# theouterlimitz/Audio-Mastering-Engine

Hardware: NVIDIA B200
Metric: audio-sec mastered/sec (x realtime) (higher is better)
Workload: dtype f64

## Files before the change

### audio_mastering_engine_b200/csrc/ame.cu

```cuda
#include <algorithm>
#include <cmath>
#include <cstdarg>
#include <cstdio>
#include <cstring>
#include <dlfcn.h>
#include <mutex>
#include <string>
#include <vector>

#include "ame_kernels.cuh"

using namespace ame;

namespace {

thread_local std::string g_err;

int fail(int code, const char *fmt, ...) {
    char buf[512];
    va_list ap;
    va_start(ap, fmt);
    vsnprintf(buf, sizeof buf, fmt, ap);
    va_end(ap);
    g_err = buf;
// ... 114 lines not shown
    std::vector<Slot> slots;
    double *d_energy = nullptr;
    int *d_chain_stats = nullptr;
    long long *d_hist = nullptr;
    int *d_hist_st = nullptr;
    int *d_peak = nullptr;
    unsigned *d_tp = nullptr;
    int *d_lim_stats = nullptr;
    int lim_guess = -1;
    ame_track_result *d_results = nullptr;
    KwJob *d_meter_kw = nullptr;
    GainJob *d_meter_peak = nullptr;
    int32_t *d_meter_tracks = nullptr;
    TrackDev *d_meter_tdev = nullptr;
    double *d_meter_energy = nullptr;
    int *d_meter_sp = nullptr;
    unsigned *d_meter_tp = nullptr;
    ame_loudness *d_loud_out = nullptr;
    ame_loudness *d_loud_any = nullptr;
    cudaStream_t s_in = nullptr, s_out = nullptr;
    std::vector<cudaEvent_t> ev_in, ev_run;
    std::vector<cudaEvent_t> ev_meter;
    bool timing = false;
    int t_step = -1, t_wave = 0;
    std::vector<cudaEvent_t> t_ev;
    std::vector<char> t_used;
    std::vector<cudaEvent_t> tl_ev;
    int tl_waves = 0;
};

namespace {

inline bool t_on(const ame_plan *p) {
    return p->timing && p->t_step >= 0 && p->t_step < kMaxTimedSteps && p->t_wave < kMaxTimedWaves;
}
inline size_t t_slot(const ame_plan *p, int kernel) {
    return ((size_t)p->t_step * kMaxTimedWaves + p->t_wave) * AME_N_KERNELS + kernel;
}
inline void t_begin(ame_plan *p, int kernel, cudaStream_t s) {
    if (t_on(p)) cudaEventRecord(p->t_ev[t_slot(p, kernel) * 2], s);
}
inline void t_end(ame_plan *p, int kernel, cudaStream_t s) {
    if (t_on(p)) {
        cudaEventRecord(p->t_ev[t_slot(p, kernel) * 2 + 1], s);
        p->t_used[t_slot(p, kernel)] = 1;
    }
}

int plan_alloc(ame_plan *p, void **ptr, size_t bytes) {
    *ptr = nullptr;
    if (bytes == 0) return AME_OK;
    cudaError_t e = dev_alloc(ptr, bytes);
    if (e != cudaSuccess) {
        *ptr = nullptr;
        return fail(AME_E_NOMEM, "device allocation of %zu bytes failed: %s", bytes, cudaGetErrorString(e));
    }
    p->allocs.push_back(*ptr);
    return AME_OK;
}

int dmalloc(ame_plan *p, void **ptr, size_t bytes) {
    const int rc = plan_alloc(p, ptr, bytes);
    if (rc == AME_OK) p->ws_bytes += bytes;
    return rc;
}

template <class T>
int upload(ame_plan *p, T **dptr, const std::vector<T> &v) {
    if (int rc = plan_alloc(p, (void **)dptr, v.size() * sizeof(T))) return rc;
    if (!v.empty()) CU(cudaMemcpy(*dptr, v.data(), v.size() * sizeof(T), cudaMemcpyHostToDevice));
    return AME_OK;
}

#define LAUNCH_CHECK(p)                                                                            \
    do {                                                                                           \
        cudaError_t e_ = cudaGetLastError();                                                       \
        if (e_ != cudaSuccess) return fail(AME_E_CUDA, "kernel launch failed: %s (%s:%d)", cudaGetErrorString(e_), __FILE__, __LINE__); \
        ++(p)->launches;                                                                           \
    } while (0)

int check_warmth(const ame_plan *p) {
    for (int t = 0; t < p->n_tracks; ++t)
        if (p->tracks[t].flags & AME_F_WARMTH) {
            const int l = p->tracks[t].warm_lut;
            if (l < 0 || l >= p->n_luts) return fail(AME_E_INVALID, "track %d needs warmth table %d but %d are set", t, l, p->n_luts);
        }
    return AME_OK;
}

struct Bufs {
    const int16_t *in = nullptr;
    int16_t *pre = nullptr, *bands = nullptr, *out = nullptr;
    uint16_t *rms = nullptr, *list = nullptr;
    int *tile_cnt = nullptr, *n_flagged = nullptr;
    GrpRec *grp = nullptr;
    double *att = nullptr;
    int64_t *hist = nullptr;
    int16_t *norm = nullptr;
    long long *lim_last = nullptr;
    LimStore lim_in{}, lim_out{};
    int *lim_need = nullptr;
};

Bufs slot_bufs(ame_plan *p, const Wave &w, const int16_t *d_in, int16_t *d_out) {
    const Slot &sl = p->slots[w.slot];
    Bufs b;
    b.in = d_in; b.out = d_out;
    b.pre = sl.pre - 2 * w.frame_lo;
    b.bands = sl.bands; b.rms = sl.rms; b.list = sl.list; b.tile_cnt = sl.tile_cnt; b.n_flagged = sl.n_flagged;
    b.grp = sl.grp; b.att = sl.att;
    b.norm = sl.norm ? sl.norm - 2 * w.frame_lo : nullptr;
    b.lim_last = sl.lim_last; b.lim_in = sl.lim_in; b.lim_out = sl.lim_out; b.lim_need = sl.lim_need;
    b.hist = (int64_t *)p->d_hist;
    return b;
}

int run_eq(ame_plan *p, const Wave &w, const int16_t *d_in, int16_t *d_pre, cudaStream_t s) {
    if (!w.eq.n) return AME_OK;
    t_begin(p, S_EQ, s);
    if (p->precision == 1)
        k_eq_f32<<<(w.eq.n + 127) / 128, 128, 0, s>>>(p->d_eq_jobs + w.eq.lo, w.eq.n, p->d_tracks, p->d_luts, d_in, d_pre);
    else
        k_eq<<<(w.eq.n + kEqBlock - 1) / kEqBlock, kEqBlock, 0, s>>>(p->d_eq_jobs + w.eq.lo, w.eq.n, p->d_tracks, p->d_luts, d_in, d_pre);
    LAUNCH_CHECK(p);
    t_end(p, S_EQ, s);
    return AME_OK;
}

int run_split(ame_plan *p, const Wave &w, const int16_t *d_pre, int16_t *d_bands, cudaStream_t s) {
    if (!w.split.n) return AME_OK;
    t_begin(p, S_SPLIT, s);
    if (w.xover_uni)
        k_band_split<true><<<(w.split.n + 127) / 128, 128, 0, s>>>(w.xover, p->d_split_jobs + w.split.lo, w.split.n, p->d_tracks, p->d_mb_delta,
                                                                   d_pre, d_bands, p->mb_frames);
    else
        k_band_split<false><<<(w.split.n + 127) / 128, 128, 0, s>>>(w.xover, p->d_split_jobs + w.split.lo, w.split.n, p->d_tracks, p->d_mb_delta,
                                                                    d_pre, d_bands, p->mb_frames);
    LAUNCH_CHECK(p);
    t_end(p, S_SPLIT, s);
    return AME_OK;
}

int chain_lanes(const ame_plan *p, int n_chains) {
    if (p->chain_warps < 0) return 1;
    if (p->chain_warps > 0) return 32 * p->chain_warps;
    if (n_chains * 2 <= p->n_sm) return 256;
    return (n_chains >= p->n_sm && p->slots.size() > 1) ? 64 : 128;
}

int run_compress(ame_plan *p, const Wave &w, const Bufs &b, cudaStream_t s) {
    if (!w.chain.n) return AME_OK;
    t_begin(p, S_FLAG, s);
    int *tile_base = b.tile_cnt + std::max(p->slot_tiles, 1);
    k_window_flag<<<w.wf.n, kWfThreads, 0, s>>>(p->d_wf_jobs + w.wf.lo, b.bands, b.rms, b.tile_cnt, b.grp);
    LAUNCH_CHECK(p);
    k_tile_prefix<<<w.chain.n, kWfThreads, 0, s>>>(p->d_chain_jobs + w.chain.lo, b.tile_cnt, tile_base, b.n_flagged);
    LAUNCH_CHECK(p);
    k_compact<<<(w.wf.n + kWfThreads / 32 - 1) / (kWfThreads / 32), kWfThreads, 0, s>>>(p->d_wf_jobs + w.wf.lo, w.wf.n, b.rms, b.tile_cnt,
                                                                                          tile_base, b.list, b.grp);
    LAUNCH_CHECK(p);
    t_end(p, S_FLAG, s);
    t_begin(p, S_CHAIN, s);
    const int lanes = chain_lanes(p, w.chain.n);
    k_att_chain<<<w.chain.n, std::max(lanes, 32), 0, s>>>(p->d_chain_jobs + w.chain.lo, b.list, b.n_flagged, p->d_tables, b.att, p->mb_frames,
                                            lanes, p->d_chain_stats + 2 * (size_t)w.chain.lo);
    LAUNCH_CHECK(p);
    t_end(p, S_CHAIN, s);
    t_begin(p, S_APPLY, s);
    k_compress_apply<<<(unsigned)((w.seg_hi - w.seg_lo + 3) / 4), 128, 0, s>>>(p->d_mb_chunks + w.mb_chunks.lo, w.mb_chunks.n, w.seg_lo, w.seg_hi,
                                                                                b.bands, b.grp, b.att, b.pre, p->mb_frames);
    LAUNCH_CHECK(p);
    t_end(p, S_APPLY, s);
    return AME_OK;
}

int run_hist(ame_plan *p, const Wave &w, const int16_t *d_pre, int64_t *d_hist, cudaStream_t s) {
    const int nt = w.track_hi - w.track_lo;
    if (nt <= 0) return AME_OK;
    CU(cudaMemsetAsync(p->d_peak + w.track_lo, 0, (size_t)nt * 4, s));
    if (w.kw.n) {
        t_begin(p, S_KW, s);
        if (w.kw_uni)
            k_kweight_energy<true><<<(w.kw.n + 127) / 128, 128, 0, s>>>(w.kw_cfg, p->d_kw_jobs + w.kw.lo, w.kw.n, p->d_tracks, p->d_tdev, d_pre,
                                                                        p->d_energy, p->d_peak);
        else
            k_kweight_energy<false><<<(w.kw.n + 127) / 128, 128, 0, s>>>(w.kw_cfg, p->d_kw_jobs + w.kw.lo, w.kw.n, p->d_tracks, p->d_tdev, d_pre,
                                                                         p->d_energy, p->d_peak);
        LAUNCH_CHECK(p);
        t_end(p, S_KW, s);
    }
    t_begin(p, S_TAIL, s);
    k_tail_peak<<<nt, 128, 0, s>>>(p->d_tracks, p->d_tdev, w.track_lo, w.track_hi, d_pre, p->d_peak);
    LAUNCH_CHECK(p);
    t_end(p, S_TAIL, s);
    CU(cudaMemsetAsync(p->d_tp + w.track_lo, 0, (size_t)nt * 4, s));
    if (w.true_peak && w.gain.n) {
        t_begin(p, S_TP, s);
        k_true_peak<<<w.gain.n, 256, 0, s>>>(p->d_gain_jobs + w.gain.lo, p->d_tracks, d_pre, p->d_tp);
        LAUNCH_CHECK(p);
        t_end(p, S_TP, s);
    }
    t_begin(p, S_HIST, s);
    k_block_hist<<<nt, 256, 0, s>>>(p->d_tdev, w.track_lo, p->d_energy, (long long *)d_hist, p->d_hist_st);
    LAUNCH_CHECK(p);
    t_end(p, S_HIST, s);
    return AME_OK;
}

int run_apply(ame_plan *p, const Wave &w, const int16_t *d_pre, int16_t *d_out, const Bufs &b, cudaStream_t s) {
    int16_t *d_norm = b.norm;
    long long *lim_last = b.lim_last;
    if (!w.gain.n) return AME_OK;
    t_begin(p, S_GAIN, s);
    if (w.limiter) CU(cudaMemsetAsync(lim_last, 0xff, (size_t)w.lim.n * sizeof(long long), s));
    k_apply_gain<<<w.gain.n, 256, 0, s>>>(p->d_gain_jobs + w.gain.lo, p->d_results, p->d_tracks, p->d_tdev, d_pre, d_out, d_norm, lim_last);
    LAUNCH_CHECK(p);
    t_end(p, S_GAIN, s);
    if (w.limiter) {
        t_begin(p, S_LIM, s);
        const GainJob *gj = p->d_lim_jobs + w.lim.lo;
        constexpr int kLimRounds = 2;
        int cap = 64;
        while (cap < p->lim_keep + 2) cap *= 2;
        const size_t smem = lim_smem_bytes(cap);
        for (int round = 0; round <= kLimRounds; ++round) {
            if (round == 0) {
                k_limiter<<<w.lim.n, 256, smem, s>>>(gj, w.lim.n, lim_last, p->d_tracks, d_norm, d_out, b.lim_in, b.lim_out, b.lim_need, 0, cap, p->lim_guess);
                LAUNCH_CHECK(p);
            }
            k_limiter<<<w.lim.n, 32, smem, s>>>(gj, w.lim.n, lim_last, p->d_tracks, d_norm, d_out, b.lim_in, b.lim_out, b.lim_need, round, cap, p->lim_guess);
            LAUNCH_CHECK(p);
            k_lim_verify<<<(w.lim.n + 3) / 4, 128, 0, s>>>(gj, w.lim.n, p->d_tracks, b.lim_in, b.lim_out, b.lim_need,
                                                             p->d_lim_stats + round);
            LAUNCH_CHECK(p);
        }
        k_lim_fallback<<<w.lim.n, 32, smem, s>>>(gj, w.lim.n, p->d_tracks, d_norm, d_out, b.lim_in, b.lim_out, b.lim_need, cap);
        LAUNCH_CHECK(p);
        t_end(p, S_LIM, s);
    }
    return AME_OK;
}

int run_gain(ame_plan *p, const Wave &w, const int16_t *d_pre, const int64_t *d_hist, int16_t *d_out, const Bufs &b, cudaStream_t s) {
    const int nt = w.track_hi - w.track_lo;
    if (nt <= 0) return AME_OK;
    t_begin(p, S_FIN, s);
    k_finalize<<<nt, 128, 0, s>>>(p->d_tracks, w.track_lo, w.track_hi, (const long long *)d_hist, p->d_hist_st, p->d_peak,
                                             p->d_tp, p->d_results);
    LAUNCH_CHECK(p);
    t_end(p, S_FIN, s);
    return run_apply(p, w, d_pre, d_out, b, s);
}

int run_meter(ame_plan *p, const Wave &w, const int16_t *buf, ame_loudness *res, cudaStream_t s) {
    if (!w.meter_tracks.n) return AME_OK;
    const int nt = w.track_hi - w.track_lo;
    CU(cudaMemsetAsync(p->d_meter_sp + w.track_lo, 0, (size_t)nt * 4, s));
    CU(cudaMemsetAsync(p->d_meter_tp + w.track_lo, 0, (size_t)nt * 4, s));
    if (w.meter_kw.n) {
        if (w.kw_uni)
            k_kweight_energy<true><<<(w.meter_kw.n + 127) / 128, 128, 0, s>>>(w.kw_cfg, p->d_meter_kw + w.meter_kw.lo, w.meter_kw.n, p->d_tracks,
                                                                              p->d_meter_tdev, buf, p->d_meter_energy, p->d_meter_sp);
        else
            k_kweight_energy<false><<<(w.meter_kw.n + 127) / 128, 128, 0, s>>>(w.kw_cfg, p->d_meter_kw + w.meter_kw.lo, w.meter_kw.n, p->d_tracks,
                                                                               p->d_meter_tdev, buf, p->d_meter_energy, p->d_meter_sp);
        LAUNCH_CHECK(p);
    }
    if (w.meter_peak.n) {
        k_meter_peak<<<w.meter_peak.n, 256, 0, s>>>(p->d_meter_peak + w.meter_peak.lo, p->d_tracks, buf, p->d_meter_tp, p->d_meter_sp);
        LAUNCH_CHECK(p);
    }
    k_meter_finalize<<<w.meter_tracks.n, 256, 0, s>>>(p->d_meter_tracks + w.meter_tracks.lo, p->d_tracks, p->d_meter_tdev, p->d_meter_energy,
                                                      p->d_meter_sp, p->d_meter_tp, res);
    LAUNCH_CHECK(p);
    return AME_OK;
}

int run_measure(ame_plan *p, const Wave &w, const Bufs &b, cudaStream_t s) {
    int rc;
    if ((rc = run_eq(p, w, b.in, b.pre, s))) return rc;
    if ((rc = run_split(p, w, b.pre, b.bands, s))) return rc;
    if ((rc = run_compress(p, w, b, s))) return rc;
    return run_hist(p, w, b.pre, b.hist, s);
}

int run_chain_of_stages(ame_plan *p, const Wave &w, const Bufs &b, cudaStream_t s) {
    int rc = run_measure(p, w, b, s);
    if (rc) return rc;
    return run_gain(p, w, b.pre, b.hist, b.out, b, s);
}

int drain(ame_plan *p, int rc) {
    (void)p;
    if (rc != AME_OK) cudaDeviceSynchronize();
    return rc;
}

}

extern "C" {

int ame_abi_version(void) { return AME_ABI_VERSION; }
size_t ame_sizeof_track_params(void) { return sizeof(ame_track_params); }
size_t ame_sizeof_track_result(void) { return sizeof(ame_track_result); }
size_t ame_sizeof_plan_options(void) { return sizeof(ame_plan_options); }
size_t ame_sizeof_loudness(void) { return sizeof(ame_loudness); }
const char *ame_last_error(void) { return g_err.c_str(); }
// ... 615 lines not shown
```

### audio_mastering_engine_b200/csrc/ame_kernels.cuh

```cuda
#pragma once
#include <cuda_runtime.h>
#include <stdint.h>
#include "ame_layout.h"

namespace ame {

constexpr unsigned kFull = 0xffffffffu;

__constant__ double c_hist_bounds[1001];
__constant__ double c_hist_energy[1000];

__device__ __forceinline__ uint4 ldg16(const uint4 *p) { return __ldg(p); }

__device__ __forceinline__ double bq_step(const ame_biquad &c, double &z0, double &z1, double x) {
    double y = fma(c.b0, x, z0);
    z0 = fma(-c.a1, y, fma(c.b1, x, z1));
    z1 = fma(-c.a2, y, c.b2 * x);
    return y;
}

__device__ __forceinline__ double i16_to_f64(int x) {
    return __hiloint2double(0x43300000, (int)(0x80000000u ^ (unsigned)x)) - 4503601774854144.0;
}

// ... 162 lines not shown
    auto fetch_lut = [&](const uint4 &q, double *l, double *r) {
        const uint32_t w[4] = {q.x, q.y, q.z, q.w};
#pragma unroll
        for (int k = 0; k < 4; ++k) {
            l[k] = __ldg(lut + (int)(int16_t)(w[k] & 0xffffu));
            r[k] = __ldg(lut + (int)(int16_t)(w[k] >> 16));
        }
    };
    if (WARM) fetch_lut(cur, lutL, lutR);
    constexpr int LAG = (SKEW && MASK != 0) ? 1 : 0;
    for (int it = 0; it < n_it + LAG; ++it) {
        uint4 nn = nxt;
        if (it + 2 < n_it) nn = ldg16(src + it + 2);
        double nL[4] = {0, 0, 0, 0}, nR[4] = {0, 0, 0, 0};
        if (WARM) fetch_lut(nxt, nL, nR);
        const int64_t g = g0f + 4 * (int64_t)(it - LAG);
        const uint32_t w[4] = {cur.x, cur.y, cur.z, cur.w};
        uint32_t o[4];
#pragma unroll
        for (int k = 0; k < 4; ++k) o[k] = frame(w[k], lutL[k], lutR[k]);
        if (it < LAG) {
        } else if (g >= job.tile_begin && g + 4 <= f_hi) {
            dst[it - LAG] = make_uint4(o[0], o[1], o[2], o[3]);
        } else {
#pragma unroll
            for (int k = 0; k < 4; ++k)
                if (g + k >= job.tile_begin && g + k < f_hi) reinterpret_cast<uint32_t *>(dst + it - LAG)[k] = o[k];
        }
        cur = nxt; nxt = nn;
#pragma unroll
        for (int k = 0; k < 4; ++k) { lutL[k] = nL[k]; lutR[k] = nR[k]; }
    }
}

#define AME_EQ_KERNEL(NAME, F, SK)                                                                                  \
__global__ void __launch_bounds__(256, 1)                                                                          \
NAME(const TileJob *__restrict__ jobs, int n_jobs, const ame_track_params *__restrict__ tracks,                    \
     const double *__restrict__ luts, const int16_t *__restrict__ in, int16_t *__restrict__ pre) {                 \
    const int j = blockIdx.x * blockDim.x + threadIdx.x;                                                           \
    if (j >= n_jobs) return;                                                                                       \
    const TileJob job = jobs[j];                                                                                   \
    if (job.tile_end <= job.tile_begin) return;                          \
    const ame_track_params *tp = tracks + job.track;                                                               \
    switch (job.variant) {                                                 \
        AME_EQ_CASE(0, F, SK) AME_EQ_CASE(1, F, SK) AME_EQ_CASE(2, F, SK) AME_EQ_CASE(3, F, SK) AME_EQ_CASE(4, F, SK)    \
        AME_EQ_CASE(5, F, SK) AME_EQ_CASE(6, F, SK) AME_EQ_CASE(7, F, SK) AME_EQ_CASE(8, F, SK) AME_EQ_CASE(9, F, SK)    \
        AME_EQ_CASE(10, F, SK) AME_EQ_CASE(11, F, SK) AME_EQ_CASE(12, F, SK) AME_EQ_CASE(13, F, SK) AME_EQ_CASE(14, F, SK) \
        AME_EQ_CASE(15, F, SK)                                                                                     \
    }                                                                                                              \
}
#define AME_EQ_CASE(M, F, SK) case M: eq_tile<M, false, F, SK>(job, tp, luts, in, pre); break; \
                              case M + 16: eq_tile<M, true, F, SK>(job, tp, luts, in, pre); break;
AME_EQ_KERNEL(k_eq, double, false)
AME_EQ_KERNEL(k_eq_f32, float, false)
#undef AME_EQ_CASE
#undef AME_EQ_KERNEL

template <bool UNI>
__global__ void __launch_bounds__(128, 3)
k_band_split(const __grid_constant__ XoverCfg xc, const TileJob *__restrict__ jobs, int n_jobs, const ame_track_params *__restrict__ tracks,
             const int64_t *__restrict__ mb_delta,
             const int16_t *__restrict__ pre, int16_t *__restrict__ bands, int64_t mb_frames) {
    const int j = blockIdx.x * blockDim.x + threadIdx.x;
    if (j >= n_jobs) return;
    const TileJob job = jobs[j];
    const ame_track_params *tp = tracks + job.track;
    const double lb0 = UNI ? xc.lb0 : tp->xlp[0].b0, la10 = UNI ? xc.la10 : tp->xlp[0].a1, la20 = UNI ? xc.la20 : tp->xlp[0].a2,
                 la11 = UNI ? xc.la11 : tp->xlp[1].a1, la21 = UNI ? xc.la21 : tp->xlp[1].a2;
    const double hb0 = UNI ? xc.hb0 : tp->xhp[0].b0, ha10 = UNI ? xc.ha10 : tp->xhp[0].a1, ha20 = UNI ? xc.ha20 : tp->xhp[0].a2,
                 ha11 = UNI ? xc.ha11 : tp->xhp[1].a1, ha21 = UNI ? xc.ha21 : tp->xhp[1].a2;
    const int64_t delta = mb_delta[job.track];
    double zl[8], zr[8];
#pragma unroll
    for (int i = 0; i < 8; ++i) { zl[i] = 0.0; zr[i] = 0.0; }
    int64_t f_lo = job.tile_begin - (int64_t)tp->warm_xover;
    if (f_lo < job.chunk_begin) f_lo = job.chunk_begin;
    const int64_t f_hi = job.tile_end;
    if (f_hi <= f_lo) return;
    const int64_t g0f = f_lo & ~(int64_t)7;
    const int n_it = (int)((f_hi - g0f + 7) >> 3);
    uint32_t *b0 = reinterpret_cast<uint32_t *>(bands) + delta;
    uint32_t *b1 = b0 + mb_frames;
    uint32_t *b2 = b1 + mb_frames;

    auto split = [&](int xm, double *z, int &p0, int &p1, int &p2) {
        const double x = i16_to_unit(xm);
        const double lo = bw_step1<1, double>(la11, la21, z[2], z[3], bw_step<1, double>(lb0, la10, la20, z[0], z[1], x));
        const double hi = bw_step1<-1, double>(ha11, ha21, z[6], z[7], bw_step<-1, double>(hb0, ha10, ha20, z[4], z[5], x));
        const double mid = __dsub_rn(__dsub_rn(x, lo), hi);
        p0 = to_pcm_f64(lo); p1 = to_pcm_f64(mid); p2 = to_pcm_f64(hi);
    };

    const uint4 *src = reinterpret_cast<const uint4 *>(pre) + (g0f >> 2);
    uint4 c0 = ldg16(src), c1 = ldg16(src + 1), n0 = make_uint4(0, 0, 0, 0), n1 = n0;
    {
        uint32_t *cw0 = reinterpret_cast<uint32_t *>(&c0), *cw1 = reinterpret_cast<uint32_t *>(&c1);
#pragma unroll
        for (int k = 0; k < 4; ++k) {
            if (g0f + k < job.chunk_begin) cw0[k] = 0;
            if (g0f + 4 + k < job.chunk_begin) cw1[k] = 0;
        }
    }
    if (n_it > 1) { n0 = ldg16(src + 2); n1 = ldg16(src + 3); }
    for (int it = 0; it < n_it; ++it) {
        uint4 m0 = n0, m1 = n1;
        if (it + 2 < n_it) { m0 = ldg16(src + 2 * it + 4); m1 = ldg16(src + 2 * it + 5); }
        const int64_t g = g0f + 8 * (int64_t)it;
        const uint32_t w[8] = {c0.x, c0.y, c0.z, c0.w, c1.x, c1.y, c1.z, c1.w};
        uint32_t o0[8], o1[8], o2[8];
#pragma unroll
        for (int k = 0; k < 8; ++k) {
            int l0, l1, l2, r0, r1, r2;
            split((int)(int16_t)(w[k] & 0xffffu), zl, l0, l1, l2);
            split((int)(int16_t)(w[k] >> 16), zr, r0, r1, r2);
            o0[k] = pack16(l0, r0); o1[k] = pack16(l1, r1); o2[k] = pack16(l2, r2);
        }
        if (g >= job.tile_begin && g + 8 <= f_hi) {
            uint4 *q0 = reinterpret_cast<uint4 *>(b0 + g), *q1 = reinterpret_cast<uint4 *>(b1 + g), *q2 = reinterpret_cast<uint4 *>(b2 + g);
            q0[0] = make_uint4(o0[0], o0[1], o0[2], o0[3]); q0[1] = make_uint4(o0[4], o0[5], o0[6], o0[7]);
            q1[0] = make_uint4(o1[0], o1[1], o1[2], o1[3]); q1[1] = make_uint4(o1[4], o1[5], o1[6], o1[7]);
            q2[0] = make_uint4(o2[0], o2[1], o2[2], o2[3]); q2[1] = make_uint4(o2[4], o2[5], o2[6], o2[7]);
        } else {
#pragma unroll
            for (int k = 0; k < 8; ++k)
                if (g + k >= job.tile_begin && g + k < f_hi) { b0[g + k] = o0[k]; b1[g + k] = o1[k]; b2[g + k] = o2[k]; }
        }
        c0 = n0; c1 = n1; n0 = m0; n1 = m1;
    }
}

__device__ __forceinline__ unsigned energy_of(uint32_t w) {
    const int l = (int16_t)(w & 0xffffu), r = (int16_t)(w >> 16);
    return (unsigned)(l * l) + (unsigned)(r * r);
}

__device__ __forceinline__ void load8(const uint32_t *__restrict__ p, int64_t idx, int64_t lo, int64_t hi, uint32_t *w) {
    if (idx >= lo && idx + 8 <= hi && ((reinterpret_cast<uintptr_t>(p + idx) & 15) == 0)) {
        const uint4 a = __ldg(reinterpret_cast<const uint4 *>(p + idx));
        const uint4 b = __ldg(reinterpret_cast<const uint4 *>(p + idx) + 1);
        w[0] = a.x; w[1] = a.y; w[2] = a.z; w[3] = a.w; w[4] = b.x; w[5] = b.y; w[6] = b.z; w[7] = b.w;
    } else {
#pragma unroll
        for (int k = 0; k < 8; ++k) w[k] = (idx + k >= lo && idx + k < hi) ? __ldg(p + idx + k) : 0u;
    }
}

__device__ __forceinline__ unsigned isqrt_ratio(unsigned long long s, unsigned n) {
    unsigned r = (unsigned)__fsqrt_rn(__fdividef((float)s, (float)n));
    if ((unsigned long long)r * r * n > s) --r;
    else if ((unsigned long long)(r + 1) * (r + 1) * n <= s) ++r;
    return r;
}

__global__ void __launch_bounds__(kWfThreads)
k_window_flag(const WfJob *__restrict__ jobs, const int16_t *__restrict__ bands, uint16_t *__restrict__ rms,
              int *__restrict__ tile_cnt, GrpRec *__restrict__ grp) {
    __shared__ long long s_scan[kWfThreads / 32];
    __shared__ unsigned long long s_head[kWfThreads / 32];
    __shared__ int s_flag[kWfThreads / 32];
    const WfJob job = jobs[blockIdx.x];
    const uint32_t *bp = reinterpret_cast<const uint32_t *>(bands) + job.plane_off;
    uint16_t *rp = rms + job.plane_off;
    const int64_t n = job.n, t0 = job.tile_begin;
    const int look = job.look;
    const int lane = threadIdx.x & 31, wid = threadIdx.x >> 5;
    const int64_t i0 = t0 + (int64_t)threadIdx.x * 8;
    uint32_t w[8], wo[8];
    load8(bp, i0, 0, n, w);
    load8(bp, i0 - look, 0, n, wo);
    unsigned long long head = 0;
    for (int64_t j = t0 - look + threadIdx.x; j < t0; j += kWfThreads)
        if (j >= 0) head += energy_of(__ldg(bp + j));
#pragma unroll
    for (int d = 16; d > 0; d >>= 1) head += __shfl_xor_sync(kFull, head, d);
    if (lane == 0) s_head[wid] = head;
    long long pre[8];
    long long run = 0;
#pragma unroll
    for (int k = 0; k < 8; ++k) {
        pre[k] = run;
        run += (long long)energy_of(w[k]) - (long long)energy_of(wo[k]);
    }
    long long incl = run;
#pragma unroll
    for (int d = 1; d < 32; d <<= 1) {
        const long long v = __shfl_up_sync(kFull, incl, d);
        if (lane >= d) incl += v;
    }
    if (lane == 31) s_scan[wid] = incl;
    __syncthreads();
    long long base = incl - run;
    unsigned long long h = 0;
#pragma unroll
    for (int q = 0; q < kWfThreads / 32; ++q) {
        if (q < wid) base += s_scan[q];
        h += s_head[q];
    }
    base += (long long)h;
    const unsigned long long thr2 = (unsigned long long)job.thr_i * job.thr_i;
    const bool never = job.thr_i > 32768u;
    uint32_t o[4] = {0, 0, 0, 0};
    unsigned m8 = 0;
    if (t0 >= look && i0 + 8 <= n) {
        const unsigned long long bound = thr2 * (unsigned long long)(2 * look);
#pragma unroll
        for (int k = 0; k < 8; ++k) {
            const unsigned long long s = (unsigned long long)(base + pre[k]);
            unsigned r = 0;
            if (!never && s >= bound) r = isqrt_ratio(s, (unsigned)(2 * look));
            m8 |= (r != 0 ? 1u : 0u) << k;
            o[k >> 1] |= (r & 0xffffu) << ((k & 1) * 16);
        }
    } else {
#pragma unroll
        for (int k = 0; k < 8; ++k) {
            const int64_t i = i0 + k;
            const long long s = base + pre[k];
            const int64_t nfr = i < look ? i : look;
            unsigned r = 0;
            if (!never && i < n && nfr > 0 && (unsigned long long)s >= thr2 * (unsigned long long)(2 * nfr))
                r = isqrt_ratio((unsigned long long)s, (unsigned)(2 * nfr));
            m8 |= (r != 0 ? 1u : 0u) << k;
            o[k >> 1] |= (r & 0xffffu) << ((k & 1) * 16);
        }
    }
    const int cnt = __popc(m8);
    int fincl = cnt;
#pragma unroll
    for (int d = 1; d < 32; d <<= 1) {
        const int v = __shfl_up_sync(kFull, fincl, d);
        if (lane >= d) fincl += v;
    }
    if (lane == 31) s_flag[wid] = fincl;
    const unsigned m1 = __shfl_down_sync(kFull, m8, 1), m2 = __shfl_down_sync(kFull, m8, 2), m3 = __shfl_down_sync(kFull, m8, 3);
    __syncthreads();
    int fbase = 0, total = 0;
#pragma unroll
    for (int q = 0; q < kWfThreads / 32; ++q) {
        if (q < wid) fbase += s_flag[q];
        total += s_flag[q];
    }
    const int rank = fbase + fincl - cnt;
    if ((threadIdx.x & 3) == 0 && i0 < n)
        grp[job.grp_begin + (i0 >> 5)] = GrpRec{m8 | (m1 << 8) | (m2 << 16) | (m3 << 24), (uint32_t)rank};
    if (m8) {
        uint16_t *dp = rp + t0 + rank;
        int slot = 0;
#pragma unroll
        for (int k = 0; k < 8; ++k)
            if (m8 & (1u << k)) dp[slot++] = (uint16_t)((o[k >> 1] >> ((k & 1) * 16)) & 0xffffu);
    }
    if (threadIdx.x == 0) tile_cnt[blockIdx.x] = total;
}

__device__ __forceinline__ double att_update(double att, double m, double inc, double dec, double tau) {
    const long long ia = __double_as_longlong(att);
    const bool above = ia > __double_as_longlong(m);
    const bool rising = ia < __double_as_longlong(tau);
    const double s = att + inc;
    const double d = att - dec;
    const double r = above ? d : m;
    return (rising && !above) ? s : r;
}

struct RmsBlk { uint32_t w[4]; };

__device__ __forceinline__ RmsBlk list_load(const uint16_t *__restrict__ lp, int64_t i, int64_t lim, bool vec) {
    RmsBlk q;
    q.w[0] = q.w[1] = q.w[2] = q.w[3] = 0;
    if (vec && i + 8 <= lim) {
        const uint4 v = __ldg(reinterpret_cast<const uint4 *>(lp + i));
        q.w[0] = v.x; q.w[1] = v.y; q.w[2] = v.z; q.w[3] = v.w;
    } else if (i < lim) {
#pragma unroll
        for (int k = 0; k < 8; ++k)
            if (i + k < lim) q.w[k >> 1] |= (uint32_t)__ldg(lp + i + k) << ((k & 1) * 16);
    }
    return q;
}

__global__ void __launch_bounds__(kWfThreads)
k_tile_prefix(const ChainJob *__restrict__ jobs, const int *__restrict__ tile_cnt, int *__restrict__ tile_base,
              int *__restrict__ n_flagged) {
    __shared__ int s_warp[kWfThreads / 32];
    const ChainJob job = jobs[blockIdx.x];
    const int n_tiles = (int)((job.n + kWfTile - 1) / kWfTile);
    const int t = threadIdx.x, lane = t & 31, wid = t >> 5;
    int carry = 0;
    for (int j0 = 0; j0 < n_tiles; j0 += kWfThreads) {
        const int j = j0 + t;
        const int c = j < n_tiles ? tile_cnt[job.tile0 + j] : 0;
        int incl = c;
#pragma unroll
        for (int d = 1; d < 32; d <<= 1) {
            const int v = __shfl_up_sync(kFull, incl, d);
            if (lane >= d) incl += v;
        }
        if (lane == 31) s_warp[wid] = incl;
        __syncthreads();
        int base = carry, total = 0;
#pragma unroll
        for (int q = 0; q < kWfThreads / 32; ++q) {
            if (q < wid) base += s_warp[q];
            total += s_warp[q];
        }
        if (j < n_tiles) tile_base[job.tile0 + j] = base + incl - c;
        carry += total;
        __syncthreads();
    }
    if (t == 0) n_flagged[blockIdx.x] = carry;
}

__global__ void __launch_bounds__(kWfThreads)
k_compact(const WfJob *__restrict__ jobs, int n_tiles, const uint16_t *__restrict__ rms, const int *__restrict__ tile_cnt,
          const int *__restrict__ tile_base, uint16_t *__restrict__ list, GrpRec *__restrict__ grp) {
    const int lane = threadIdx.x & 31;
    const int tile = blockIdx.x * (kWfThreads / 32) + (threadIdx.x >> 5);
    if (tile >= n_tiles) return;
    const WfJob job = jobs[tile];
    const int cnt = tile_cnt[tile], base = tile_base[tile];
    if (base) {
        const int64_t frames = min((int64_t)kWfTile, job.n - job.tile_begin);
        const int ng = (int)((frames + 31) >> 5);
        GrpRec *gr = grp + job.grp_begin + (job.tile_begin >> 5);
        for (int g = lane; g < ng; g += 32) gr[g].base += (uint32_t)base;
    }
    const uint16_t *rp = rms + job.plane_off + job.tile_begin;
    uint16_t *lp = list + job.plane_off + base;
    for (int j = lane; j < cnt; j += 32) lp[j] = rp[j];
}


__device__ __forceinline__ void list_entries(AttEntry *e, const AttEntry *tbl, const RmsBlk &q) {
#pragma unroll
    for (int k = 0; k < 8; ++k) {
        const unsigned r = (q.w[k >> 1] >> ((k & 1) * 16)) & 0xffffu;
        asm("ld.global.nc.v4.f64 {%0,%1,%2,%3}, [%4];" : "=d"(e[k].m), "=d"(e[k].inc), "=d"(e[k].dec), "=d"(e[k].tau) : "l"(tbl + r));
    }
}

struct SegSum {
    long long margin;
    long long at_p;
    long long lo, hi;
    int64_t p;
    int exp0;
    bool open;
    bool ok;
};

__device__ __forceinline__ void segsum_begin(SegSum &u, double start) {
    u.margin = 0x7fffffffffffffffLL; u.at_p = 0; u.lo = 0; u.hi = -1; u.p = 0;
    u.exp0 = (int)(__double_as_longlong(start) >> 52);
    u.open = true; u.ok = u.exp0 > 0;
}

template <bool DUAL>
__device__ __forceinline__ bool list_step8(const AttEntry *e, double *al, int64_t i, int64_t lim, bool avec, double &a, double &b,
                                           SegSum &u, double &max_m, double &sum_dec) {
    double o[8];
#pragma unroll
    for (int k = 0; k < 8; ++k) {
        if (!DUAL) { max_m = fmax(max_m, e[k].m); sum_dec += e[k].dec; }
        if (DUAL && u.open && i + k < lim) {
            const long long ib = __double_as_longlong(b), im = __double_as_longlong(e[k].m);
            if (ib > im) {
                u.margin = min(u.margin, ib - im);
                const long long id = __double_as_longlong(e[k].dec);
                if (id != 0) {
                    const int ed = (int)(id >> 52);
                    const long long mant = (id & 0xfffffffffffffLL) | (ed ? (1LL << 52) : 0LL);
                    if ((ed ? ed : 1) + (__ffsll(mant) - 1) == u.exp0 - 1) u.ok = false;
                }
                ++u.p;
            } else {
                u.open = false;
                u.at_p = ib; u.lo = __double_as_longlong(e[k].tau); u.hi = im;
                if ((int)(ib >> 52) != u.exp0) u.ok = false;
            }
        }
        b = att_update(b, e[k].m, e[k].inc, e[k].dec, e[k].tau);
        if (DUAL) a = att_update(a, e[k].m, e[k].inc, e[k].dec, e[k].tau);
        o[k] = b;
    }
    if (avec && i + 8 <= lim) {
        double2 *d = reinterpret_cast<double2 *>(al + i);
        d[0] = make_double2(o[0], o[1]); d[1] = make_double2(o[2], o[3]);
        d[2] = make_double2(o[4], o[5]); d[3] = make_double2(o[6], o[7]);
    } else {
#pragma unroll
        for (int k = 0; k < 8; ++k)
            if (i + k < lim) al[i + k] = o[k];
    }
    return DUAL && __double_as_longlong(a) == __double_as_longlong(b);
}

template <bool DUAL>
__device__ __forceinline__ bool list_walk(const uint16_t *lp, const AttEntry *tbl, double *al, int64_t b0, int64_t b1, bool vec,
                                          bool avec, double a, double &b, SegSum &u, double &max_m, double &sum_dec) {
    if (b0 >= b1) return false;
    RmsBlk r0 = list_load(lp, b0, b1, vec), r1 = list_load(lp, b0 + 8, b1, vec);
    AttEntry ea[8], eb[8];
    list_entries(ea, tbl, r0);
    for (int64_t i = b0; i < b1; i += 16) {
        r0 = list_load(lp, i + 16, b1, vec);
// ... 867 lines not shown
```

Before: 932,100.

## Process each window-flag tile with a single warp looping over rows

Rewrites k_window_flag so that one warp handles a whole tile by looping in 256-sample rows. Prefix sums and flag counts carry across rows in registers instead of going through shared memory and __syncthreads. The next row's loads are prefetched while the current row is scanned. A monotone threshold test also skips the isqrt when the running sum is below the bound. The risks are a serial loop per warp, fewer blocks per tile, and a new 'wide' fallback path for the -32768 sample case.

New measurement: 958,800 (median of 6 runs). 2.9% higher.

```diff
diff --git a/audio_mastering_engine_b200/csrc/ame.cu b/audio_mastering_engine_b200/csrc/ame.cu
--- a/audio_mastering_engine_b200/csrc/ame.cu
+++ b/audio_mastering_engine_b200/csrc/ame.cu
@@ -290,7 +290,8 @@
     if (!w.chain.n) return AME_OK;
     t_begin(p, S_FLAG, s);
     int *tile_base = b.tile_cnt + std::max(p->slot_tiles, 1);
-    k_window_flag<<<w.wf.n, kWfThreads, 0, s>>>(p->d_wf_jobs + w.wf.lo, b.bands, b.rms, b.tile_cnt, b.grp);
+    k_window_flag<<<(w.wf.n + kWfWarps - 1) / kWfWarps, kWfWarps * 32, 0, s>>>(p->d_wf_jobs + w.wf.lo, w.wf.n, b.bands, b.rms,
+                                                                              b.tile_cnt, b.grp);
     LAUNCH_CHECK(p);
     k_tile_prefix<<<w.chain.n, kWfThreads, 0, s>>>(p->d_chain_jobs + w.chain.lo, b.tile_cnt, tile_base, b.n_flagged);
     LAUNCH_CHECK(p);
diff --git a/audio_mastering_engine_b200/csrc/ame_kernels.cuh b/audio_mastering_engine_b200/csrc/ame_kernels.cuh
--- a/audio_mastering_engine_b200/csrc/ame_kernels.cuh
+++ b/audio_mastering_engine_b200/csrc/ame_kernels.cuh
@@ -338,105 +338,111 @@
     return r;
 }
 
-__global__ void __launch_bounds__(kWfThreads)
-k_window_flag(const WfJob *__restrict__ jobs, const int16_t *__restrict__ bands, uint16_t *__restrict__ rms,
+constexpr int kWfWarps = 4;
+
+__global__ void __launch_bounds__(kWfWarps * 32, 6)
+k_window_flag(const WfJob *__restrict__ jobs, int n_tiles, const int16_t *__restrict__ bands, uint16_t *__restrict__ rms,
               int *__restrict__ tile_cnt, GrpRec *__restrict__ grp) {
-    __shared__ long long s_scan[kWfThreads / 32];
-    __shared__ unsigned long long s_head[kWfThreads / 32];
-    __shared__ int s_flag[kWfThreads / 32];
-    const WfJob job = jobs[blockIdx.x];
+    const int lane = threadIdx.x & 31;
+    const int tile = blockIdx.x * kWfWarps + (threadIdx.x >> 5);
+    if (tile >= n_tiles) return;
+    const WfJob job = jobs[tile];
     const uint32_t *bp = reinterpret_cast<const uint32_t *>(bands) + job.plane_off;
     uint16_t *rp = rms + job.plane_off;
     const int64_t n = job.n, t0 = job.tile_begin;
     const int look = job.look;
-    const int lane = threadIdx.x & 31, wid = threadIdx.x >> 5;
-    const int64_t i0 = t0 + (int64_t)threadIdx.x * 8;
-    uint32_t w[8], wo[8];
-    load8(bp, i0, 0, n, w);
-    load8(bp, i0 - look, 0, n, wo);
-    unsigned long long head = 0;
-    for (int64_t j = t0 - look + threadIdx.x; j < t0; j += kWfThreads)
-        if (j >= 0) head += energy_of(__ldg(bp + j));
-#pragma unroll
-    for (int d = 16; d > 0; d >>= 1) head += __shfl_xor_sync(kFull, head, d);
-    if (lane == 0) s_head[wid] = head;
-    long long pre[8];
-    long long run = 0;
-#pragma unroll
-    for (int k = 0; k < 8; ++k) {
-        pre[k] = run;
-        run += (long long)energy_of(w[k]) - (long long)energy_of(wo[k]);
-    }
-    long long incl = run;
-#pragma unroll
-    for (int d = 1; d < 32; d <<= 1) {
-        const long long v = __shfl_up_sync(kFull, incl, d);
-        if (lane >= d) incl += v;
-    }
-    if (lane == 31) s_scan[wid] = incl;
-    __syncthreads();
-    long long base = incl - run;
-    unsigned long long h = 0;
-#pragma unroll
-    for (int q = 0; q < kWfThreads / 32; ++q) {
-        if (q < wid) base += s_scan[q];
-        h += s_head[q];
-    }
-    base += (long long)h;
     const unsigned long long thr2 = (unsigned long long)job.thr_i * job.thr_i;
     const bool never = job.thr_i > 32768u;
-    uint32_t o[4] = {0, 0, 0, 0};
-    unsigned m8 = 0;
-    if (t0 >= look && i0 + 8 <= n) {
-        const unsigned long long bound = thr2 * (unsigned long long)(2 * look);
+    const unsigned long long bound = thr2 * (unsigned long long)(2 * look);
+
+    uint32_t w[8], wo[8];
+    load8(bp, t0 + 8 * lane, 0, n, w);
+    load8(bp, t0 + 8 * lane - look, 0, n, wo);
+    unsigned long long head = 0;
+    for (int64_t j = t0 - look + lane; j < t0; j += 32)
+        if (j >= 0) head += energy_of(__ldg(bp + j));
+#pragma unroll
+    for (int d = 16; d > 0; d >>= 1) head += __shfl_xor_sync(kFull, head, d);
+    long long carry = (long long)head;
+    int fcarry = 0;
+#pragma unroll 1
+    for (int64_t r0 = t0; r0 < t0 + kWfTile; r0 += 256) {
+        const int64_t i0 = r0 + 8 * lane;
+        int d[8];
+        long long dsum = 0;
 #pragma unroll
         for (int k = 0; k < 8; ++k) {
-            const unsigned long long s = (unsigned long long)(base + pre[k]);
-            unsigned r = 0;
-            if (!never && s >= bound) r = isqrt_ratio(s, (unsigned)(2 * look));
-            m8 |= (r != 0 ? 1u : 0u) << k;
-            o[k >> 1] |= (r & 0xffffu) << ((k & 1) * 16);
-        }
-    } else {
-#pragma unroll
-        for (int k = 0; k < 8; ++k) {
-            const int64_t i = i0 + k;
-            const long long s = base + pre[k];
-            const int64_t nfr = i < look ? i : look;
-            unsigned r = 0;
-            if (!never && i < n && nfr > 0 && (unsigned long long)s >= thr2 * (unsigned long long)(2 * nfr))
-                r = isqrt_ratio((unsigned long long)s, (unsigned)(2 * nfr));
-            m8 |= (r != 0 ? 1u : 0u) << k;
-            o[k >> 1] |= (r & 0xffffu) << ((k & 1) * 16);
-        }
-    }
-    const int cnt = __popc(m8);
-    int fincl = cnt;
-#pragma unroll
-    for (int d = 1; d < 32; d <<= 1) {
-        const int v = __shfl_up_sync(kFull, fincl, d);
-        if (lane >= d) fincl += v;
-    }
-    if (lane == 31) s_flag[wid] = fincl;
-    const unsigned m1 = __shfl_down_sync(kFull, m8, 1), m2 = __shfl_down_sync(kFull, m8, 2), m3 = __shfl_down_sync(kFull, m8, 3);
-    __syncthreads();
-    int fbase = 0, total = 0;
-#pragma unroll
-    for (int q = 0; q < kWfThreads / 32; ++q) {
-        if (q < wid) fbase += s_flag[q];
-        total += s_flag[q];
-    }
-    const int rank = fbase + fincl - cnt;
-    if ((threadIdx.x & 3) == 0 && i0 < n)
-        grp[job.grp_begin + (i0 >> 5)] = GrpRec{m8 | (m1 << 8) | (m2 << 16) | (m3 << 24), (uint32_t)rank};
-    if (m8) {
-        uint16_t *dp = rp + t0 + rank;
-        int slot = 0;
-#pragma unroll
-        for (int k = 0; k < 8; ++k)
-            if (m8 & (1u << k)) dp[slot++] = (uint16_t)((o[k >> 1] >> ((k & 1) * 16)) & 0xffffu);
-    }
-    if (threadIdx.x == 0) tile_cnt[blockIdx.x] = total;
+            const long long dk = (long long)energy_of(w[k]) - (long long)energy_of(wo[k]);
+            dsum += dk;
+            d[k] = (int)dk;
+        }
+        bool wide = false;
+#pragma unroll
+        for (int k = 0; k < 8; ++k) wide |= w[k] == 0x80008000u;
+        uint32_t wn[8], won[8];
+        if (r0 + 256 < t0 + kWfTile) {
+            load8(bp, i0 + 256, 0, n, wn);
+            load8(bp, i0 + 256 - look, 0, n, won);
+        }
+        long long incl = dsum;
+#pragma unroll
+        for (int s = 1; s < 32; s <<= 1) {
+            const long long v = __shfl_up_sync(kFull, incl, s);
+            if (lane >= s) incl += v;
+        }
+        const long long entry = carry + incl - dsum;
+        carry += __shfl_sync(kFull, incl, 31);
+
+        uint32_t o[4] = {0, 0, 0, 0};
+        unsigned m8 = 0;
+        if (!never && !wide && i0 >= look && i0 + 8 <= n) {
+            long long t = entry - (long long)bound;
+#pragma unroll
+            for (int k = 0; k < 8; ++k) {
+                if (t >= 0) {
+                    const unsigned rv = isqrt_ratio((unsigned long long)(t + (long long)bound), (unsigned)(2 * look));
+                    m8 |= 1u << k;
+                    o[k >> 1] |= rv << ((k & 1) * 16);
+                }
+                t += d[k];
+            }
+        } else if (!never) {
+            long long s = entry;
+#pragma unroll
+            for (int k = 0; k < 8; ++k) {
+                const int64_t i = i0 + k;
+                const int64_t nfr = i < look ? i : look;
+                unsigned rv = 0;
+                if (i < n && nfr > 0 && (unsigned long long)s >= thr2 * (unsigned long long)(2 * nfr))
+                    rv = isqrt_ratio((unsigned long long)s, (unsigned)(2 * nfr));
+                m8 |= (rv != 0 ? 1u : 0u) << k;
+                o[k >> 1] |= (rv & 0xffffu) << ((k & 1) * 16);
+                s += (long long)energy_of(w[k]) - (long long)energy_of(wo[k]);
+            }
+        }
+        const int cnt = __popc(m8);
+        int fincl = cnt;
+#pragma unroll
+        for (int s = 1; s < 32; s <<= 1) {
+            const int v = __shfl_up_sync(kFull, fincl, s);
+            if (lane >= s) fincl += v;
+        }
+        const int rank = fcarry + fincl - cnt;
+        fcarry += __shfl_sync(kFull, fincl, 31);
+        const unsigned m1 = __shfl_down_sync(kFull, m8, 1), m2 = __shfl_down_sync(kFull, m8, 2), m3 = __shfl_down_sync(kFull, m8, 3);
+        if ((lane & 3) == 0 && i0 < n)
+            grp[job.grp_begin + (i0 >> 5)] = GrpRec{m8 | (m1 << 8) | (m2 << 16) | (m3 << 24), (uint32_t)rank};
+        if (m8) {
+            uint16_t *dp = rp + t0 + rank;
+            int slot = 0;
+#pragma unroll
+            for (int k = 0; k < 8; ++k)
+                if (m8 & (1u << k)) dp[slot++] = (uint16_t)((o[k >> 1] >> ((k & 1) * 16)) & 0xffffu);
+        }
+#pragma unroll
+        for (int k = 0; k < 8; ++k) { w[k] = wn[k]; wo[k] = won[k]; }
+    }
+    if (lane == 0) tile_cnt[tile] = fcarry;
 }
 
 __device__ __forceinline__ double att_update(double att, double m, double inc, double dec, double tau) {
```
